# NTU-CompHydroMet-Lab/P2I-GAN-benchmark

Hardware: AMD Instinct MI355X
Metric: train frames/sec (128x128x16) (higher is better)
Workload: dtype f32

## Files before the change

### p2i-gan-benchmark_amd/csrc/conv.hip

```cpp
#include "conv_dma.h"

namespace p2i {


template <int MB, int NPIX, int WAVES_M, int CK>
__global__ __launch_bounds__(256) void patch_gemm_kernel(const PatchGeom g) {
  extern __shared__ __attribute__((aligned(16))) float smem[];
  constexpr int WAVES_N = 4 / WAVES_M;
  constexpr int TM = MB / (32 * WAVES_M);
  constexpr int TN = NPIX / (32 * WAVES_N);
  static_assert(TM >= 1 && TN >= 1, "tile too small");
  float* lw = smem;
  float* lp = smem + g.ntaps * CK * MB;

  const int tid = threadIdx.x, lane = tid & 63, wave = tid >> 6;
  const int wm = wave / WAVES_N, wn = wave % WAVES_N;
  const int l31 = lane & 31, lhi = lane >> 5;

  int tile = blockIdx.x;
  const int tw = tile % g.ntw; tile /= g.ntw;
  const int th = tile % g.nth; tile /= g.nth;
  const int tt = tile % g.ntt;
  const int tb = tile / g.ntt;
  const int j0b = tb << g.ljb, j0t = tt << g.ljt, j0h = th << g.ljh, j0w = tw << g.ljw;
// ... 104 lines not shown
          if (g.res) v += g.res[di];
          if (g.mask_y) v = act_grad(v, g.mask_y[di], g.mask_act);
          g.dst[di] = v;
        }
      }
    }
  }
}


typedef void (*patch_fn)(const PatchGeom);
template <int MB, int NPIX, int WM, int CK>
static int launch_patch(const PatchGeom& g, dim3 grid, size_t lds, hipStream_t s) {
  auto k = patch_gemm_kernel<MB, NPIX, WM, CK>;
  static bool attr_set = false;
  if (!attr_set) {
    (void)hipFuncSetAttribute((const void*)k, hipFuncAttributeMaxDynamicSharedMemorySize, 160 * 1024);
    attr_set = true;
  }
  P2I_LAUNCH(k, grid, dim3(256), lds, s, g);
  return launch_status();
}

static int dispatch_patch_dma(const TileCfg& c, int KG, const PatchGeom& g, dim3 grid, size_t lds, hipStream_t s) {
  int rc = dispatch_patch_dma_g0(c, KG, g, grid, lds, s);
  if (rc == -1) rc = dispatch_patch_dma_g1(c, KG, g, grid, lds, s);
  if (rc == -1) rc = dispatch_patch_dma_g2(c, KG, g, grid, lds, s);
  if (rc == -1) rc = dispatch_patch_dma_g3(c, KG, g, grid, lds, s);
  if (rc != -1) return rc;
  set_error("no DMA kernel instance for tile cfg %d %d %d %d kg %d", c.MB, c.NPIX, c.WM, c.CK, KG);
  return P2I_EINVAL;
}

static int dispatch_patch(const TileCfg& c, const PatchGeom& g, dim3 grid, size_t lds, hipStream_t s) {
#define P2I_CASE(mb_, npix_, wm_, ck_) \
  if (c.MB == mb_ && c.NPIX == npix_ && c.WM == wm_ && c.CK == ck_) return launch_patch<mb_, npix_, wm_, ck_>(g, grid, lds, s);
  P2I_CASE(128, 256, 2, 8)
  P2I_CASE(64, 256, 1, 8)
  P2I_CASE(64, 128, 2, 8)
  P2I_CASE(32, 128, 1, 8)
  P2I_CASE(128, 256, 2, 4)
  P2I_CASE(64, 256, 1, 4)
  P2I_CASE(64, 128, 2, 4)
  P2I_CASE(32, 128, 1, 4)
  P2I_CASE(128, 256, 2, 2)
  P2I_CASE(64, 256, 1, 2)
  P2I_CASE(64, 128, 2, 2)
  P2I_CASE(32, 128, 1, 2)
#undef P2I_CASE
  set_error("no kernel instance for tile cfg %d %d %d %d", c.MB, c.NPIX, c.WM, c.CK);
  return P2I_EINVAL;
}


static thread_local int g_last_plan[6] = {0, 0, 0, 0, 0, 0};

static int run_patch_gemm(PatchGeom g, const ClassSpec& cs, hipStream_t s);

static int run_patch_gemm_classes(PatchGeom g, const ClassSpec* css, int ncls, hipStream_t s) {
  if (g.src_y != nullptr || ncls > MAX_CLASSES) return 1;
  if (const X6Ctx& xc = x6_ctx(); xc.wb != nullptr) {
    bool all = true;
    for (int q = 0; q < ncls && all; ++q) all = run_patch_gemm_x6c(g, css[q], xc.wb, xc.ntaps_w, nullptr, s, true) == 0;
    if (all) {
      for (int q = 0; q < ncls; ++q)
        if (const int rc = run_patch_gemm_x6c(g, css[q], xc.wb, xc.ntaps_w, g_last_plan, s)) return rc == 1 ? P2I_EINVAL : rc;
      return P2I_OK;
    }
  }
  const ClassSpec& c0s = css[0];
  g.mT = c0s.mT; g.mH = c0s.mH; g.mW = c0s.mW;
  g.oT = c0s.oT; g.oH = c0s.oH; g.oW = c0s.oW;
  int lo[MAX_CLASSES][3], rng[3] = {0, 0, 0}, mx[3] = {0, 0, 0}, max_taps = 0;
  long long total_pix = 0;
  for (int q = 0; q < ncls; ++q) {
    const ClassSpec& cs = css[q];
    int hi[3] = {0, 0, 0};
    lo[q][0] = lo[q][1] = lo[q][2] = 0;
    for (int i = 0; i < cs.ntaps; ++i) {
      const int d[3] = {cs.dt[i], cs.dh[i], cs.dw[i]};
      for (int k = 0; k < 3; ++k) {
        if (i == 0 || d[k] < lo[q][k]) lo[q][k] = d[k];
        if (i == 0 || d[k] > hi[k]) hi[k] = d[k];
      }
    }
    for (int k = 0; k < 3; ++k) if (hi[k] - lo[q][k] > rng[k]) rng[k] = hi[k] - lo[q][k];
    if (cs.nT > mx[0]) mx[0] = cs.nT;
    if (cs.nH > mx[1]) mx[1] = cs.nH;
    if (cs.nW > mx[2]) mx[2] = cs.nW;
    if (cs.ntaps > max_taps) max_taps = cs.ntaps;
    total_pix += (long long)g.B * (cs.nT > 0 ? cs.nT : 0) * (cs.nH > 0 ? cs.nH : 0) * (cs.nW > 0 ? cs.nW : 0);
  }
  if (mx[0] <= 0 || mx[1] <= 0 || mx[2] <= 0) return P2I_OK;
  if (max_taps == 0) max_taps = 1;
  g.ntaps = max_taps;
  static const int cand[5][3] = {{128, 256, 2}, {64, 256, 1}, {128, 128, 2}, {64, 128, 2}, {32, 128, 1}};
  int best = -1, best_ck = 0;
  long long best_score = -1;
  PatchGeom bg = g;
  size_t best_lds = 0;
  dim3 best_grid;
  for (int ci = 0; ci < 5; ++ci) {
    const int MBc = cand[ci][0], NP = cand[ci][1];
    if (MBc > 32 && g.Cm <= MBc / 2) continue;
    int jb, jt, jh, jw;
    pick_tile_dims(NP, g.B, mx[0], mx[1], mx[2], jb, jt, jh, jw);
    PatchGeom t = g;
    t.ljb = ilog2(jb); t.ljt = ilog2(jt); t.ljh = ilog2(jh); t.ljw = ilog2(jw);
    t.eT = (jt - 1) * g.mT + rng[0] + 1;
    t.eH = (jh - 1) * g.mH + rng[1] + 1;
    t.eW = (jw - 1) * g.mW + rng[2] + 1;
    static const int v4_off = getenv("P2I_CONV_V4") ? (atoi(getenv("P2I_CONV_V4")) == 0) : 0;
    bool same_lo_w = true;
    for (int q = 1; q < ncls; ++q) same_lo_w = same_lo_w && lo[q][2] == lo[0][2];
    t.v4 = (!v4_off && same_lo_w && (g.sW & 3) == 0 && ((jw * g.mW) & 3) == 0) ? 1 : 0;
    t.v4sh = 0;
    if (t.v4) {
      t.v4sh = ((lo[0][2] % 4) + 4) % 4;
      t.eW = (t.eW + t.v4sh + 3) & ~3;
      t.eW4 = t.eW >> 2;
    }
    t.eWp = t.eW;
    t.eth = t.eT * t.eH;
    t.rpc = jb * t.eth;
    t.CSl = t.rpc * t.eW;
    t.CS = t.CSl;
    t.G4 = t.CSl >> 2;
    static const int force_ck16 = getenv("P2I_CONV_CK16") ? atoi(getenv("P2I_CONV_CK16")) : 0;
    for (int CKc = ((max_taps <= 4 || ((force_ck16 || g.Ck >= 256) && max_taps == 9 && MBc <= 64)) ? 16 : 8); CKc >= 2; CKc >>= 1) {
      if (g.Ck >= CKc ? (g.Ck % CKc != 0) : (CKc != 2 && g.Ck * 2 <= CKc)) continue;
      if (CKc == 2 && !(MBc == 64 && NP == 128) && !(MBc == 32)) continue;
      if ((CKc == 4 || CKc == 16) && MBc == 128 && NP == 128) continue;
      const int PT = CKc * t.CSl;
      if (PT >= 65536 || t.CSl >= 65536) continue;
      const int PTp = t.v4 ? (((PT >> 2) + 63) & ~63) * 4 : (PT + 63) & ~63;
      const int nwrows = max_taps * CKc;
      const size_t WSZ = (size_t)((nwrows * (MBc / 4) + 63) & ~63) * 4;
      const size_t lds = sizeof(float) * (((nwrows + 63) & ~63) + (size_t)PTp + 2 * (WSZ + PTp));
      if (lds > 160 * 1024) continue;
      const long long nb = (long long)ceil_div(g.Cm, MBc) * ((total_pix + NP - 1) / NP);
      long long score = (nb >= 256 ? 1000000000ll : nb * 1000000ll) + (long long)MBc * NP * 10 + CKc + (lds <= 80 * 1024 ? 5 : 0);
      if (score > best_score) {
        best_score = score; best = ci; best_ck = CKc; best_lds = lds;
        bg = t; bg.PT = PT;
        bg.ntt = ceil_div(mx[0], jt); bg.nth = ceil_div(mx[1], jh); bg.ntw = ceil_div(mx[2], jw);
        best_grid = dim3((unsigned)(ceil_div(g.B, jb) * bg.ntt * bg.nth * bg.ntw), (unsigned)ceil_div(g.Cm, MBc), (unsigned)ncls);
      }
      break;
    }
  }
  const unsigned long long sbytes = 4ull * g.B * g.Ck * g.sT * g.sH * g.sW;
  if (best < 0 || sbytes >= 0xF0000000ull) return 1;
  TileCfg c{cand[best][0], cand[best][1], cand[best][2], best_ck};
  bg.mg_csl = magic_u16(bg.CSl); bg.mg_ew = magic_u16(bg.eW);
  bg.mg_rpc = magic_u16(bg.rpc); bg.mg_eth = magic_u16(bg.eth); bg.mg_eh = magic_u16(bg.eH);
  if (bg.v4) { bg.mg_g4 = magic_u16(bg.G4); bg.mg_ew4 = magic_u16(bg.eW4); }
  bg.src_bytes = (unsigned)sbytes;
  bg.wp_bytes = g.wp_bytes;
  bg.nclass = ncls;
  for (int q = 0; q < ncls; ++q) {
    const ClassSpec& cs = css[q];
    ClassGeom& cgm = bg.cls[q];
    cgm.nT = cs.nT; cgm.nH = cs.nH; cgm.nW = cs.nW;
    cgm.pT = cs.pT; cgm.pH = cs.pH; cgm.pW = cs.pW;
    cgm.bT = lo[q][0]; cgm.bH = lo[q][1]; cgm.bW = lo[q][2];
    cgm.ntaps = cs.ntaps;
    for (int i = 0; i < cs.ntaps; ++i) {
      cgm.tap_w[i] = cs.tw[i];
      cgm.tap_off[i] = ((cs.dt[i] - lo[q][0]) * bg.eH + (cs.dh[i] - lo[q][1])) * bg.eW + (cs.dw[i] - lo[q][2]);
    }
  }
  bg.nT = css[0].nT; bg.nH = css[0].nH; bg.nW = css[0].nW;
  bg.pT = css[0].pT; bg.pH = css[0].pH; bg.pW = css[0].pW;
  bg.bT = lo[0][0]; bg.bH = lo[0][1]; bg.bW = lo[0][2];
  for (int i = 0; i < css[0].ntaps; ++i) { bg.tap_w[i] = bg.cls[0].tap_w[i]; bg.tap_off[i] = bg.cls[0].tap_off[i]; }
  if (bg.v4) {
    bg.bW -= bg.v4sh;
    for (int i = 0; i < css[0].ntaps; ++i) bg.tap_off[i] += bg.v4sh;
    for (int q = 0; q < ncls; ++q) {
      bg.cls[q].bW -= bg.v4sh;
      for (int i = 0; i < css[q].ntaps; ++i) bg.cls[q].tap_off[i] += bg.v4sh;
    }
  }
  if (ncls == 1) bg.ntaps = css[0].ntaps;
  const long long nb = (long long)best_grid.x * best_grid.y * best_grid.z;
  const int acc_regs = (c.MB / 32) * (c.NPIX / 32) / 4 * 16;
  const size_t red_bytes = (size_t)4 * acc_regs * 64 * 4;
  static const int kg27 = getenv("P2I_CONV_KG27") ? atoi(getenv("P2I_CONV_KG27")) : 1;
  const bool kg_27 = kg27 && max_taps == 27 && c.CK == 4 && ncls == 1;
  const int KG = ((nb <= 320 || (c.CK == 16 && max_taps == 9) || kg_27) && (c.CK >= 8 || kg_27) && c.MB <= 64 && red_bytes <= best_lds) ? 2 : 1;
  g_last_plan[0] = c.MB; g_last_plan[1] = c.NPIX; g_last_plan[2] = c.WM; g_last_plan[3] = c.CK;
  g_last_plan[4] = ncls > 1 ? 0 : ((max_taps == 9 && (c.CK <= 8 || KG == 2)) ? 9 : (max_taps == 1 ? 1 : ((max_taps == 27 && (c.CK == 4 || (c.CK < 4 && KG == 1))) ? 27 : 0)));
  g_last_plan[5] = KG;
  return dispatch_patch_dma(c, KG, bg, best_grid, best_lds, s);
}

static int run_patch_gemm(PatchGeom g, const ClassSpec& cs, hipStream_t s) {
  if (cs.nT <= 0 || cs.nH <= 0 || cs.nW <= 0) return P2I_OK;
  {
    const int rc = run_patch_gemm_classes(g, &cs, 1, s);
    if (rc != 1) return rc;
  }
  g.nT = cs.nT; g.nH = cs.nH; g.nW = cs.nW;
  g.mT = cs.mT; g.mH = cs.mH; g.mW = cs.mW;
  g.oT = cs.oT; g.oH = cs.oH; g.oW = cs.oW; g.pT = cs.pT; g.pH = cs.pH; g.pW = cs.pW;
  g.ntaps = cs.ntaps;
  g.nclass = 1;
  int lo[3] = {0, 0, 0}, hi[3] = {0, 0, 0};
  for (int i = 0; i < cs.ntaps; ++i) {
    const int d[3] = {cs.dt[i], cs.dh[i], cs.dw[i]};
    for (int k = 0; k < 3; ++k) {
      if (i == 0 || d[k] < lo[k]) lo[k] = d[k];
      if (i == 0 || d[k] > hi[k]) hi[k] = d[k];
    }
  }
  g.bT = lo[0]; g.bH = lo[1]; g.bW = lo[2];

  TileCfg c;
  c.CK = (g.Ck == 1) ? 2 : (cs.ntaps > 9 ? 4 : 8);
  if (g.Ck < c.CK && g.Ck > 1) c.CK = (g.Ck >= 4) ? 4 : 2;
  c.MB = g.Cm > 64 ? 128 : (g.Cm > 32 ? 64 : 32);
  c.NPIX = 256;
  const long long total_pix = (long long)g.B * cs.nT * cs.nH * cs.nW;
  auto nblocks = [&](const TileCfg& t) { return (long long)ceil_div(g.Cm, t.MB) * ((total_pix + t.NPIX - 1) / t.NPIX); };
  const long long want = 512;
  while (nblocks(c) < want) {
    if (c.MB == 128) { c.MB = 64; continue; }
    if (c.NPIX == 256) { c.NPIX = 128; continue; }
    if (c.MB == 64 && g.Cm > 32) { c.MB = 32; continue; }
    break;
  }
  if (c.MB == 128) { c.NPIX = 256; c.WM = 2; }
  else if (c.MB == 64) { c.WM = (c.NPIX == 256) ? 1 : 2; }
  else { c.NPIX = 128; c.WM = 1; }

  for (int attempt = 0; attempt < 4; ++attempt) {
    int jb, jt, jh, jw;
    pick_tile_dims(c.NPIX, g.B, cs.nT, cs.nH, cs.nW, jb, jt, jh, jw);
    g.ljb = ilog2(jb); g.ljt = ilog2(jt); g.ljh = ilog2(jh); g.ljw = ilog2(jw);
    g.eT = (jt - 1) * cs.mT + (hi[0] - lo[0]) + 1;
    g.eH = (jh - 1) * cs.mH + (hi[1] - lo[1]) + 1;
    g.eW = (jw - 1) * cs.mW + (hi[2] - lo[2]) + 1;
    g.eWp = g.eW | 1;
    g.eth = g.eT * g.eH;
    g.rpc = jb * g.eth;
    g.CS = g.rpc * g.eWp;
    g.mg_rpc = magic_u16(g.rpc); g.mg_eth = magic_u16(g.eth); g.mg_eh = magic_u16(g.eH);
    const size_t lds = sizeof(float) * ((size_t)cs.ntaps * c.CK * c.MB + (size_t)c.CK * g.CS);
    if (lds > 160 * 1024 || c.CK * g.rpc >= 65536) {
      if (c.CK > 2) { c.CK /= 2; continue; }
      if (c.NPIX == 256) { c.NPIX = 128; c.WM = (c.MB == 64) ? 2 : (c.MB == 128 ? 2 : 1); if (c.MB == 128) c.MB = 64; continue; }
      set_error("conv tile does not fit LDS (%zu bytes)", lds);
      return P2I_ELDS;
    }
    for (int i = 0; i < cs.ntaps; ++i) {
      g.tap_w[i] = cs.tw[i];
      g.tap_off[i] = ((cs.dt[i] - lo[0]) * g.eH + (cs.dh[i] - lo[1])) * g.eWp + (cs.dw[i] - lo[2]);
    }
    g.ntt = ceil_div(cs.nT, jt); g.nth = ceil_div(cs.nH, jh); g.ntw = ceil_div(cs.nW, jw);
    const int ntb = ceil_div(g.B, jb);
    dim3 grid((unsigned)(ntb * g.ntt * g.nth * g.ntw), (unsigned)ceil_div(g.Cm, c.MB));
    g_last_plan[0] = c.MB; g_last_plan[1] = c.NPIX; g_last_plan[2] = c.WM; g_last_plan[3] = c.CK; g_last_plan[4] = -1; g_last_plan[5] = 0;
    return dispatch_patch(c, g, grid, lds, s);
  }
  set_error("conv tile selection failed");
  return P2I_ELDS;
}

}

using namespace p2i;

#ifdef P2I_STAMP
namespace p2i { __device__ unsigned long long* p2i_stamp_buf = nullptr; }
extern "C" int p2i_debug_set_stamp(unsigned long long* buf) {
  return (int)hipMemcpyToSymbol(HIP_SYMBOL(p2i::p2i_stamp_buf), &buf, sizeof(buf));
}
#endif

extern "C" int p2i_conv_last_plan(int* out6) {
  if (!out6) return P2I_EINVAL;
  for (int i = 0; i < 6; ++i) out6[i] = g_last_plan[i];
  return P2I_OK;
}

extern "C" int p2i_conv_fwd(const p2i_conv_desc* d, const float* x, const float* wp, const float* bias,
                            const float* residual, float* y, int act, void* stream) {
  if (int e = check_desc(d)) return e;
  P2I_REQUIRE(x && wp && y, "null pointer");
  if (d->Cin == 1 && residual == nullptr && x6_ctx().wb == nullptr) {
    const int rc = c1_fwd(d, x, wp, bias, y, act, (hipStream_t)stream);
    if (rc != 1) { g_last_plan[0] = 32; g_last_plan[1] = 64; g_last_plan[2] = 1; g_last_plan[3] = 2; g_last_plan[4] = 27; g_last_plan[5] = 1; return rc; }
  }
  if (d->Cout == 1 && residual == nullptr) {
    const int rc = o1_fwd(d, x, wp, bias, y, act, (hipStream_t)stream);
    if (rc != 1) { g_last_plan[0] = 1; g_last_plan[1] = 64; g_last_plan[2] = 8; g_last_plan[3] = 1; g_last_plan[4] = 9; g_last_plan[5] = 3; return rc; }
  }
  PatchGeom g{};
  g.src = x; g.src_y = nullptr; g.wp = wp; g.bias = bias; g.res = residual; g.dst = y; g.act_epi = act; g.act_pro = P2I_ACT_NONE;
  g.B = d->B; g.Ck = d->Cin; g.Cm = d->Cout; g.CmPad = (d->Cout + 31) / 32 * 32;
  g.wp_bytes = 4u * (unsigned)(d->kt * d->kh * d->kw) * g.Ck * g.CmPad;
  g.sT = d->Ti; g.sH = d->Hi; g.sW = d->Wi; g.dT = d->To; g.dH = d->Ho; g.dW = d->Wo;
  ClassSpec cs{};
  cs.nT = d->To; cs.nH = d->Ho; cs.nW = d->Wo;
  cs.mT = d->st; cs.mH = d->sh; cs.mW = d->sw;
  cs.oT = cs.oH = cs.oW = 1; cs.pT = cs.pH = cs.pW = 0;
  int n = 0;
  for (int a = 0; a < d->kt; ++a)
    for (int b = 0; b < d->kh; ++b)
      for (int c = 0; c < d->kw; ++c) {
        cs.tw[n] = (short)n; cs.dt[n] = a - d->pt; cs.dh[n] = b - d->ph; cs.dw[n] = c - d->pw; ++n;
      }
  cs.ntaps = n;
  return run_patch_gemm(g, cs, (hipStream_t)stream);
}

extern "C" int p2i_conv_dgrad(const p2i_conv_desc* d, const float* dy, const float* y_act, int act,
                              const float* wp_d, const float* dx_add, const float* mask_y, int mask_act,
                              float* dx, void* stream) {
  if (int e = check_desc(d)) return e;
  P2I_REQUIRE(dy && wp_d && dx, "null pointer");
  PatchGeom g{};
  g.src = dy; g.src_y = y_act; g.wp = wp_d; g.bias = nullptr; g.res = dx_add; g.dst = dx; g.act_epi = P2I_ACT_NONE; g.act_pro = y_act ? act : P2I_ACT_NONE;
  g.mask_y = mask_y; g.mask_act = mask_y ? mask_act : P2I_ACT_NONE;
  P2I_REQUIRE(!(mask_y && y_act), "dgrad: use either the act'(y) prologue or the epilogue mask");
  if (d->Cin == 1 && !y_act && d->kt * d->kh * d->kw * d->Cout * 4 <= 64 * 1024)
    return c1_dgrad(d, dy, wp_d, dx_add, mask_y, mask_act, dx, (hipStream_t)stream);
  g.B = d->B; g.Ck = d->Cout; g.Cm = d->Cin; g.CmPad = (d->Cin + 31) / 32 * 32;
  g.wp_bytes = 4u * (unsigned)(d->kt * d->kh * d->kw) * g.Ck * g.CmPad;
  g.sT = d->To; g.sH = d->Ho; g.sW = d->Wo; g.dT = d->Ti; g.dH = d->Hi; g.dW = d->Wi;
  ClassSpec css[MAX_CLASSES];
  int ncls = 0;
  const bool mergeable = d->st * d->sh * d->sw <= MAX_CLASSES;
  for (int ct = 0; ct < d->st; ++ct)
    for (int chh = 0; chh < d->sh; ++chh)
      for (int cw = 0; cw < d->sw; ++cw) {
        ClassSpec cs{};
        cs.nT = (d->Ti - ct + d->st - 1) / d->st;
        cs.nH = (d->Hi - chh + d->sh - 1) / d->sh;
        cs.nW = (d->Wi - cw + d->sw - 1) / d->sw;
        cs.mT = cs.mH = cs.mW = 1;
        cs.oT = d->st; cs.oH = d->sh; cs.oW = d->sw; cs.pT = ct; cs.pH = chh; cs.pW = cw;
        int n = 0;
// ... 96 lines not shown
```

### p2i-gan-benchmark_amd/csrc/conv_common.h

```cpp
#pragma once
#include "common.h"

namespace p2i {

typedef float f32x16 __attribute__((ext_vector_type(16)));
constexpr int MAX_TAPS = 27;

typedef __attribute__((address_space(3))) void lds_void;
typedef int v4i32 __attribute__((ext_vector_type(4)));

__device__ __forceinline__ v4i32 make_rsrc(const void* p, unsigned bytes) {
  const unsigned long long a = (unsigned long long)p;
  v4i32 r;
  r[0] = __builtin_amdgcn_readfirstlane((int)(unsigned)a);
  r[1] = __builtin_amdgcn_readfirstlane((int)(unsigned)(a >> 32));
  r[2] = __builtin_amdgcn_readfirstlane((int)bytes);
  r[3] = 0x00020000;
  return r;
}
__device__ __forceinline__ unsigned lds_base(const float* shared_array) {
  return (unsigned)(size_t)(const lds_void*)shared_array;
}
__device__ __forceinline__ void dma_b32(const v4i32 rsrc, unsigned lds_addr, int voff, int soff) {
  const unsigned la = __builtin_amdgcn_readfirstlane(lds_addr);
// ... 7 lines not shown
  const int so = __builtin_amdgcn_readfirstlane(soff);
  unsigned keep;
  asm volatile("s_nop 4\n\ts_mov_b32 %0, m0\n\ts_mov_b32 m0, %2\n\ts_nop 0\n\tbuffer_load_dwordx4 %1, %3, %4 offen lds\n\ts_mov_b32 m0, %0"
               : "=&s"(keep) : "v"(voff), "s"(la), "s"(rsrc), "s"(so) : "memory");
}
__device__ __forceinline__ void dma_wait_all() { asm volatile("s_waitcnt vmcnt(0)" ::: "memory"); }


__device__ __forceinline__ void epilogue_tile16(const f32x16& acc, int o_base, int lhi, int Cm, bool pv, size_t pos_off, size_t chan_stride,
                                                const float* __restrict__ bias, int act_epi, const float* __restrict__ res,
                                                const float* __restrict__ mask_y, int mask_act, float* __restrict__ dst,
                                                bool atomic_out = false) {
#pragma unroll
  for (int h8 = 0; h8 < 2; ++h8) {
    int di[8];
    bool ok[8];
#pragma unroll
    for (int k = 0; k < 8; ++k) {
      const int r = h8 * 8 + k;
      const int o = o_base + (r & 3) + 8 * (r >> 2) + 4 * lhi;
      ok[k] = pv && o < Cm;
      di[k] = ok[k] ? (int)((size_t)o * chan_stride + pos_off) : 0;
    }
    float rv[8], mv[8];
    if (res) {
#pragma unroll
      for (int k = 0; k < 8; ++k) rv[k] = res[di[k]];
    }
    if (mask_y) {
#pragma unroll
      for (int k = 0; k < 8; ++k) mv[k] = mask_y[di[k]];
    }
#pragma unroll
    for (int k = 0; k < 8; ++k) {
      const int r = h8 * 8 + k;
      const int o = o_base + (r & 3) + 8 * (r >> 2) + 4 * lhi;
      float v = acc[r];
      if (bias) v += bias[o < Cm ? o : 0];
      v = act_apply(v, act_epi);
      if (res) v += rv[k];
      if (mask_y) v = act_grad(v, mv[k], mask_act);
      if (ok[k]) {
        if (atomic_out) atomicAdd(dst + di[k], v);
        else dst[di[k]] = v;
      }
    }
    __builtin_amdgcn_sched_barrier(0);
  }
}

typedef float f32x4e __attribute__((ext_vector_type(4)));
__device__ __forceinline__ void epilogue_tile16_v4(const f32x16& acc, float* __restrict__ tile_lds, int o_base, int lane, int Cm,
                                                   size_t pos4_off, bool pv4, size_t chan_stride,
                                                   const float* __restrict__ bias, int act_epi, const float* __restrict__ res,
                                                   const float* __restrict__ mask_y, int mask_act, float* __restrict__ dst, bool atomic_out = false) {
  constexpr int PITCH = 36;
  const int l31 = lane & 31, lhi = lane >> 5;
#pragma unroll
  for (int r = 0; r < 16; ++r) tile_lds[((r & 3) + 8 * (r >> 2) + 4 * lhi) * PITCH + l31] = acc[r];
  __builtin_amdgcn_fence(__ATOMIC_RELEASE, "wavefront");
  __builtin_amdgcn_wave_barrier();
  const int p4 = (lane & 7) * 4;
  int di[4];
  bool ok[4];
  f32x4e v[4], rv[4], mv[4];
#pragma unroll
  for (int k = 0; k < 4; ++k) {
    const int ch = k * 8 + (lane >> 3);
    const int o = o_base + ch;
    ok[k] = pv4 && o < Cm;
    di[k] = ok[k] ? (int)((size_t)o * chan_stride + pos4_off) : 0;
    v[k] = *reinterpret_cast<const f32x4e*>(tile_lds + ch * PITCH + p4);
  }
  if (res) {
#pragma unroll
    for (int k = 0; k < 4; ++k) rv[k] = *reinterpret_cast<const f32x4e*>(res + di[k]);
  }
  if (mask_y) {
#pragma unroll
    for (int k = 0; k < 4; ++k) mv[k] = *reinterpret_cast<const f32x4e*>(mask_y + di[k]);
  }
#pragma unroll
  for (int k = 0; k < 4; ++k) {
    const int o = o_base + k * 8 + (lane >> 3);
    const float bv = bias ? bias[o < Cm ? o : 0] : 0.f;
#pragma unroll
    for (int e = 0; e < 4; ++e) {
      float x = act_apply(v[k][e] + bv, act_epi);
      if (res) x += rv[k][e];
      if (mask_y) x = act_grad(x, mv[k][e], mask_act);
      v[k][e] = x;
    }
    if (ok[k]) {
      if (atomic_out) {
#pragma unroll
        for (int e = 0; e < 4; ++e) atomicAdd(dst + di[k] + e, v[k][e]);
      } else {
        *reinterpret_cast<f32x4e*>(dst + di[k]) = v[k];
      }
    }
  }
  __builtin_amdgcn_wave_barrier();
}

__device__ __forceinline__ void epilogue_pair16(const f32x16& acc0, const f32x16& acc1, int o_base, int lhi, int Cm, bool pv, size_t pos_off,
                                                size_t chan_stride, const float* __restrict__ res, const float* __restrict__ mask_y,
                                                int mask_act, float* __restrict__ dst, bool atomic_out = false) {
  typedef float f32x2e __attribute__((ext_vector_type(2)));
#pragma unroll
  for (int h4 = 0; h4 < 4; ++h4) {
    int di[4];
    bool ok[4];
#pragma unroll
    for (int k = 0; k < 4; ++k) {
      const int r = h4 * 4 + k;
      const int o = o_base + (r & 3) + 8 * (r >> 2) + 4 * lhi;
      ok[k] = pv && o < Cm;
      di[k] = ok[k] ? (int)((size_t)o * chan_stride + pos_off) : 0;
    }
    f32x2e rv[4], mv[4];
    if (res) {
#pragma unroll
      for (int k = 0; k < 4; ++k) rv[k] = *reinterpret_cast<const f32x2e*>(res + di[k]);
    }
    if (mask_y) {
#pragma unroll
      for (int k = 0; k < 4; ++k) mv[k] = *reinterpret_cast<const f32x2e*>(mask_y + di[k]);
    }
#pragma unroll
    for (int k = 0; k < 4; ++k) {
      const int r = h4 * 4 + k;
      f32x2e v;
      v[0] = acc0[r]; v[1] = acc1[r];
      if (res) { v[0] += rv[k][0]; v[1] += rv[k][1]; }
      if (mask_y) { v[0] = act_grad(v[0], mv[k][0], mask_act); v[1] = act_grad(v[1], mv[k][1], mask_act); }
      if (ok[k]) {
        if (atomic_out) { atomicAdd(dst + di[k], v[0]); atomicAdd(dst + di[k] + 1, v[1]); }
        else *reinterpret_cast<f32x2e*>(dst + di[k]) = v;
      }
    }
    __builtin_amdgcn_sched_barrier(0);
  }
}

static inline void pick_tile_dims(int NPIX, int B, int nT, int nH, int nW, int& jb, int& jt, int& jh, int& jw) {
  jw = pow2_ceil(nW); if (jw > 32) jw = 32;
  int rem = NPIX / jw;
  jh = pow2_ceil(nH); if (jh > rem) jh = rem;
  rem /= jh;
  jt = pow2_ceil(nT); if (jt > rem) jt = rem;
  rem /= jt;
  jb = rem;
  (void)B;
}


static inline int check_desc(const p2i_conv_desc* d) {
  P2I_REQUIRE(d != nullptr, "null conv desc");
  P2I_REQUIRE(d->B > 0 && d->Cin > 0 && d->Cout > 0, "bad channel/batch dims");
  P2I_REQUIRE(d->kt >= 1 && d->kh >= 1 && d->kw >= 1 && d->kt * d->kh * d->kw <= MAX_TAPS, "kernel taps > %d", MAX_TAPS);
  P2I_REQUIRE(d->st >= 1 && d->sh >= 1 && d->sw >= 1, "bad stride");
  P2I_REQUIRE(d->To == (d->Ti + 2 * d->pt - d->kt) / d->st + 1, "To inconsistent");
  P2I_REQUIRE(d->Ho == (d->Hi + 2 * d->ph - d->kh) / d->sh + 1, "Ho inconsistent");
  P2I_REQUIRE(d->Wo == (d->Wi + 2 * d->pw - d->kw) / d->sw + 1, "Wo inconsistent");
  const long long nin = (long long)d->B * d->Cin * d->Ti * d->Hi * d->Wi;
  const long long nout = (long long)d->B * d->Cout * d->To * d->Ho * d->Wo;
  P2I_REQUIRE(nin < (1ll << 31) && nout < (1ll << 31), "tensor too large for 32-bit indexing");
  return P2I_OK;
}


struct ClassGeom {
  int nT, nH, nW, pT, pH, pW, bT, bH, bW, ntaps;
  short tap_w[MAX_TAPS];
  int tap_off[MAX_TAPS];
};
constexpr int MAX_CLASSES = 8;

struct PatchGeom {
  const float* src;
  const float* src_y;
  const float* wp;
  const float* bias;
  const float* res;
  float* dst;
  int act_epi;
  int act_pro;
  int B, Ck, Cm, CmPad;
  int sT, sH, sW;
  int dT, dH, dW;
  int nT, nH, nW;
  int mT, mH, mW;
  int oT, oH, oW;
  int pT, pH, pW;
  int bT, bH, bW;
  int eT, eH, eW, eWp;
  int ljb, ljt, ljh, ljw;
  int ntt, nth, ntw;
  int ntaps;
  int CS;
  int rpc, eth;
  unsigned mg_rpc, mg_eth, mg_eh;
  short tap_w[MAX_TAPS];
  int tap_off[MAX_TAPS];
  const float* mask_y;
  int mask_act;
  int CSl;
  int PT;
  unsigned src_bytes, wp_bytes;
  unsigned mg_csl, mg_ew;
  int v4, v4sh;
  int eW4, G4;
  unsigned mg_g4, mg_ew4;
  const uint16_t* wb;
  unsigned wb_bytes;
  int ntaps_w;
  int TG, NTP, R;
  int ksplit;
  int pair_w;
  int nclass;
  ClassGeom cls[MAX_CLASSES];
};

struct ClassSpec {
  int nT, nH, nW;
  int mT, mH, mW;
  int oT, oH, oW, pT, pH, pW;
  int ntaps;
  short tw[MAX_TAPS];
  int dt[MAX_TAPS], dh[MAX_TAPS], dw[MAX_TAPS];
};

struct X6Ctx { const uint16_t* wb; int ntaps_w; };
X6Ctx& x6_ctx();

int run_patch_gemm_x6c(PatchGeom g, const ClassSpec& cs, const uint16_t* wb, int ntaps_w, int* plan6, hipStream_t s, bool dry = false);
int run_patch_gemm_x6c_fused(PatchGeom g, const ClassSpec* css, int ncls, const uint16_t* wb, int ntaps_w, int* plan6, hipStream_t s, bool dry = false);
bool x6c_would_take(const p2i_conv_desc* d, bool dgrad, int act_epi);

int run_patch_gemm_fused(PatchGeom g, const ClassSpec* css, int ncls, int* plan6, hipStream_t s);

int c1_dgrad(const p2i_conv_desc* d, const float* dy, const float* wp_d, const float* add, const float* mask_y, int mask_act,
             float* dx, hipStream_t s);
int c1_wgrad(const p2i_conv_desc* d, const float* x, const float* dy, float* dwp, float* dbias, hipStream_t s);
int c1_fwd(const p2i_conv_desc* d, const float* x, const float* wp, const float* bias, float* y, int act, hipStream_t s);
int o1_fwd(const p2i_conv_desc* d, const float* x, const float* wp, const float* bias, float* y, int act, hipStream_t s);

}
```

### p2i-gan-benchmark_amd/csrc/conv_dma.h

```cpp
#pragma once
#include "conv_common.h"

namespace p2i {

struct TileCfg { int MB, NPIX, WM, CK; };

#ifdef P2I_STAMP
extern __device__ unsigned long long* p2i_stamp_buf;
#endif

template <int MB, int NPIX, int WAVES_M, int CK, int NT, int KG>
__global__ __launch_bounds__(256 * KG) void patch_gemm_dma_kernel(const PatchGeom g) {
  extern __shared__ __attribute__((aligned(16))) float smem[];
  constexpr int WAVES_N = 4 / WAVES_M;
  constexpr int TM = MB / (32 * WAVES_M);
  constexpr int TN = NPIX / (32 * WAVES_N);
  constexpr int V = MB / 4;
  const bool multi = g.nclass > 1;
  const ClassGeom& cg = g.cls[multi ? blockIdx.z : 0];
  const int c_nT = multi ? cg.nT : g.nT, c_nH = multi ? cg.nH : g.nH, c_nW = multi ? cg.nW : g.nW;
  const int c_pT = multi ? cg.pT : g.pT, c_pH = multi ? cg.pH : g.pH, c_pW = multi ? cg.pW : g.pW;
  const int c_bT = multi ? cg.bT : g.bT, c_bH = multi ? cg.bH : g.bH, c_bW = multi ? cg.bW : g.bW;
  const int c_ntaps = multi ? cg.ntaps : g.ntaps;
  const short* c_tap_w = multi ? cg.tap_w : g.tap_w;
  const int* c_tap_off = multi ? cg.tap_off : g.tap_off;
  const int nwrows = g.ntaps * CK;
  const int WSZ = ((nwrows * V + 63) & ~63) * 4;
  const int PT4p = ((g.PT >> 2) + 63) & ~63;
  const int PTp = g.v4 ? PT4p * 4 : (g.PT + 63) & ~63;
  int* wtab = reinterpret_cast<int*>(smem);
  const int wtab_sz = (nwrows + 63) & ~63;
  int* ptab = wtab + wtab_sz;
  float* buf0 = smem + wtab_sz + PTp;
  const int BUFSZ = WSZ + PTp;

  constexpr int NTH = 256 * KG;
#ifdef P2I_STAMP
  unsigned long long st_entry;
  asm volatile("s_memtime %0\n\ts_waitcnt lgkmcnt(0)" : "=s"(st_entry) :: "memory");
#endif
  const int tid = threadIdx.x, lane = tid & 63, wave = (tid >> 6) & 3, kg = tid >> 8;
  const int wm = wave / WAVES_N, wn = wave % WAVES_N;
  const int l31 = lane & 31, lhi = lane >> 5;

  int tile = blockIdx.x;
  const int tw = tile % g.ntw; tile /= g.ntw;
  const int th = tile % g.nth; tile /= g.nth;
  const int tt = tile % g.ntt;
  const int tb = tile / g.ntt;
  const int j0b = tb << g.ljb, j0t = tt << g.ljt, j0h = th << g.ljh, j0w = tw << g.ljw;
  const int o0 = blockIdx.y * MB;
  const int JWm = (1 << g.ljw) - 1, JHm = (1 << g.ljh) - 1, JTm = (1 << g.ljt) - 1;
  const int sHW = g.sH * g.sW;
  const int src_t0 = j0t * g.mT + c_bT, src_h0 = j0h * g.mH + c_bH, src_w0 = j0w * g.mW + c_bW;

  for (int r = tid; r < wtab_sz; r += NTH) {
    int off = -4;
    if (r < nwrows) {
      const int tap = r / CK, c = r - tap * CK;
      if (tap < c_ntaps && c < g.Ck && o0 < g.CmPad) off = ((c_tap_w[tap] * g.Ck + c) * g.CmPad + o0) * 4;
    }
    wtab[r] = off;
  }
  if (g.v4) {
    for (int e = tid; e < PT4p; e += NTH) {
      int off = -16;
      if (e < (g.PT >> 2)) {
        const int c = fast_div(e, g.mg_g4);
        int rem = e - c * g.G4;
        const int row = g.eW4 == 1 ? rem : fast_div(rem, g.mg_ew4);
        const int g4 = rem - row * g.eW4;
        const int jb = fast_div(row, g.mg_eth);
        int r2 = row - jb * g.eth;
        const int et = fast_div(r2, g.mg_eh);
        const int eh = r2 - et * g.eH;
        const int b = j0b + jb, t = src_t0 + et, h = src_h0 + eh, w = src_w0 + 4 * g4;
        if (b < g.B && c < g.Ck && (unsigned)t < (unsigned)g.sT && (unsigned)h < (unsigned)g.sH && (unsigned)w < (unsigned)g.sW)
          off = ((((b * g.Ck + c) * g.sT + t) * sHW) + h * g.sW + w) * 4;
      }
      ptab[e] = off;
    }
  } else
  for (int e = tid; e < PTp; e += NTH) {
    int off = -4;
    if (e < g.PT) {
      const int c = fast_div(e, g.mg_csl);
      int rem = e - c * g.CSl;
      const int row = fast_div(rem, g.mg_ew);
      const int ew = rem - row * g.eW;
      const int jb = fast_div(row, g.mg_eth);
      int r2 = row - jb * g.eth;
      const int et = fast_div(r2, g.mg_eh);
      const int eh = r2 - et * g.eH;
      const int b = j0b + jb, t = src_t0 + et, h = src_h0 + eh, w = src_w0 + ew;
      if (b < g.B && c < g.Ck && (unsigned)t < (unsigned)g.sT && (unsigned)h < (unsigned)g.sH && (unsigned)w < (unsigned)g.sW)
        off = ((((b * g.Ck + c) * g.sT + t) * sHW) + h * g.sW + w) * 4;
    }
    ptab[e] = off;
  }

  int lane_base[TN];
#pragma unroll
  for (int f = 0; f < TN; ++f) {
    const int pix = (wn * TN + f) * 32 + l31;
    const int jw = pix & JWm;
    const int jh = (pix >> g.ljw) & JHm;
    const int jt = (pix >> (g.ljw + g.ljh)) & JTm;
    const int jb = pix >> (g.ljw + g.ljh + g.ljt);
    lane_base[f] = ((jb * g.eT + jt * g.mT) * g.eH + jh * g.mH) * g.eW + jw * g.mW + lhi * g.CSl;
  }
  f32x16 acc[TM][TN];
#pragma unroll
  for (int i = 0; i < TM; ++i)
#pragma unroll
    for (int f = 0; f < TN; ++f)
#pragma unroll
      for (int r = 0; r < 16; ++r) acc[i][f][r] = 0.f;

  const v4i32 rs_src = make_rsrc(g.src, g.src_bytes);
  const v4i32 rs_w = make_rsrc(g.wp, g.wp_bytes);
  const unsigned smem_la = lds_base(smem);
  const int buf0_off = (int)(buf0 - smem);
  const int chan_bytes = g.sT * sHW * 4;
  const int wbase = tid & ~63;
  const int nwv = nwrows * V;
  __syncthreads();

  constexpr int RW = 10, RP = 4;
  const int nwq = (((nwv + 63) & ~63) + NTH - 1) / NTH;
  const int npq = g.v4 ? (PT4p + NTH - 1) / NTH : RP + 1;
  const bool reg_issue = nwq <= RW && npq <= RP;
  int wv[RW], pv[RP];
  if (reg_issue) {
#pragma unroll
    for (int i = 0; i < RW; ++i) {
      const int f = i * NTH + tid;
      int voff = -4;
      if (i < nwq && f < nwv) {
        const int row = f / V, col4 = f - row * V;
        const int base = wtab[row];
        voff = base < 0 ? -4 : base + col4 * 16;
      }
      wv[i] = voff;
    }
#pragma unroll
    for (int i = 0; i < RP; ++i) {
      const int e = i * NTH + tid;
      pv[i] = (i < npq && e < PT4p) ? ptab[e] : -16;
    }
  }
  auto issue = [&](int c0, int bufoff) {
    const int w_soff = c0 * g.CmPad * 4;
    if (reg_issue) {
      const int p_soff = c0 * chan_bytes, pbo = bufoff + WSZ;
#pragma unroll
      for (int i = 0; i < RW; ++i)
        if (i < nwq && i * NTH + wbase < ((nwv + 63) & ~63))
          dma_b128(rs_w, smem_la + 4u * (bufoff + (i * NTH + wbase) * 4), wv[i], w_soff);
#pragma unroll
      for (int i = 0; i < RP; ++i)
        if (i < npq && i * NTH + wbase < PT4p)
          dma_b128(rs_src, smem_la + 4u * (pbo + (i * NTH + wbase) * 4), pv[i], p_soff);
      return;
    }
    for (int f0 = 0; f0 < nwv; f0 += NTH) {
      const int f = f0 + tid;
      int voff = -4;
      if (f < nwv) {
        const int row = f / V, col4 = f - row * V;
        const int base = wtab[row];
        voff = base < 0 ? -4 : base + col4 * 16;
      }
      if (f0 + wbase < ((nwv + 63) & ~63))
        dma_b128(rs_w, smem_la + 4u * (bufoff + (f0 + wbase) * 4), voff, w_soff);
    }
    const int pbo = bufoff + WSZ;
    const int p_soff = c0 * chan_bytes;
    if (g.v4) {
      for (int e0 = 0; e0 < PT4p; e0 += NTH) {
        const int e = e0 + tid;
        const int voff = e < PT4p ? ptab[e] : -16;
        if (e0 + wbase < PT4p)
          dma_b128(rs_src, smem_la + 4u * (pbo + (e0 + wbase) * 4), voff, p_soff);
      }
    } else
    for (int e0 = 0; e0 < PTp; e0 += NTH) {
      const int e = e0 + tid;
      const int voff = e < PTp ? ptab[e] : -4;
      if (e0 + wbase < PTp)
        dma_b32(rs_src, smem_la + 4u * (pbo + e0 + wbase), voff, p_soff);
    }
  };

  int toffs[NT > 0 ? NT : 1];
  if constexpr (NT > 0) {
#pragma unroll
    for (int t = 0; t < NT; ++t) toffs[t] = c_tap_off[t];
  }
  const int nchunks = (g.Ck + CK - 1) / CK;
#ifdef P2I_STAMP
  unsigned long long st_wait = 0, st_bar = 0, st_issue = 0, st_mfma = 0, st_t0, st_t1;
#define P2I_STAMP_NOW(v) do { __builtin_amdgcn_sched_barrier(0); asm volatile("s_memtime %0\n\ts_waitcnt lgkmcnt(0)" : "=s"(v) :: "memory"); __builtin_amdgcn_sched_barrier(0); } while (0)
  unsigned long long st_begin; P2I_STAMP_NOW(st_begin);
#endif
  issue(0, buf0_off);
  for (int k = 0; k < nchunks; ++k) {
#ifdef P2I_STAMP
    P2I_STAMP_NOW(st_t0);
#endif
    dma_wait_all();
#ifdef P2I_STAMP
    P2I_STAMP_NOW(st_t1); st_wait += st_t1 - st_t0;
#endif
    __syncthreads();
#ifdef P2I_STAMP
    P2I_STAMP_NOW(st_t0); st_bar += st_t0 - st_t1;
#endif
    float* cur = buf0 + (k & 1) * BUFSZ;
    if (k + 1 < nchunks) issue((k + 1) * CK, buf0_off + ((k + 1) & 1) * BUFSZ);
#ifdef P2I_STAMP
    P2I_STAMP_NOW(st_t1); st_issue += st_t1 - st_t0;
#endif
    const float* lw = cur + lhi * MB + wm * TM * 32 + l31;
    const float* lp = cur + WSZ;
    constexpr int NCP = CK / 2 / KG;
    float a[NCP][TM], bv[NCP][TN], an[NCP][TM], bn[NCP][TN];
    auto load_tap = [&](int tap, int toff, float (&aa)[NCP][TM], float (&bb)[NCP][TN]) {
#pragma unroll
      for (int cp = 0; cp < NCP; ++cp) {
#pragma unroll
        for (int i = 0; i < TM; ++i) aa[cp][i] = lw[tap * CK * MB + (kg * NCP + cp) * 2 * MB + i * 32];
#pragma unroll
        for (int f = 0; f < TN; ++f) bb[cp][f] = lp[lane_base[f] + toff + (kg * NCP + cp) * 2 * g.CSl];
      }
    };
    auto mfma_tap = [&](const float (&aa)[NCP][TM], const float (&bb)[NCP][TN]) {
#pragma unroll
      for (int cp = 0; cp < NCP; ++cp)
#pragma unroll
        for (int i = 0; i < TM; ++i)
#pragma unroll
          for (int f = 0; f < TN; ++f)
            acc[i][f] = __builtin_amdgcn_mfma_f32_32x32x2f32(aa[cp][i], bb[cp][f], acc[i][f], 0, 0, 0);
    };
    if constexpr (NT > 0) {
      load_tap(0, toffs[0], a, bv);
#pragma unroll
      for (int tap = 0; tap < NT; tap += 2) {
        if (tap + 1 < NT) load_tap(tap + 1, toffs[tap + 1 < NT ? tap + 1 : 0], an, bn);
        __builtin_amdgcn_sched_barrier(0);
        mfma_tap(a, bv);
        __builtin_amdgcn_sched_barrier(0);
        if (tap + 1 < NT) {
          if (tap + 2 < NT) load_tap(tap + 2, toffs[tap + 2 < NT ? tap + 2 : 0], a, bv);
          __builtin_amdgcn_sched_barrier(0);
          mfma_tap(an, bn);
          __builtin_amdgcn_sched_barrier(0);
        }
      }
    } else {
      const int nt = c_ntaps;
      if (nt > 0) load_tap(0, c_tap_off[0], a, bv);
// ... 107 lines not shown
```

Baseline: 11690.

## Add stride-2 conv replanning with lean tile dims and parity-split LDS patch layout

For single-class stride-2 (mW==2) convolutions, the host planner now re-picks tile dimensions to minimise the staged halo footprint. It can also store the LDS input patch with even and odd columns split and a padded row pitch chosen to reduce bank conflicts. The kernel's patch-table builder and lane base addressing are updated to use the padded pitch and the parity column mapping. The default mode (3) enables only the lean tile selection without parity, and keeps the vector path. This trades some extra host planning work and LDS footprint for less redundant staging and fewer LDS bank conflicts.

```diff
diff --git a/p2i-gan-benchmark_amd/csrc/conv.hip b/p2i-gan-benchmark_amd/csrc/conv.hip
--- a/p2i-gan-benchmark_amd/csrc/conv.hip
+++ b/p2i-gan-benchmark_amd/csrc/conv.hip
@@ -280,7 +280,8 @@
   const unsigned long long sbytes = 4ull * g.B * g.Ck * g.sT * g.sH * g.sW;
   if (best < 0 || sbytes >= 0xF0000000ull) return 1;
   TileCfg c{cand[best][0], cand[best][1], cand[best][2], best_ck};
-  bg.mg_csl = magic_u16(bg.CSl); bg.mg_ew = magic_u16(bg.eW);
+  bg.mg_csl = magic_u16(bg.CSl); bg.mg_ew = magic_u16(bg.eWp);
+  bg.par = 0; bg.eWh = 0;
   bg.mg_rpc = magic_u16(bg.rpc); bg.mg_eth = magic_u16(bg.eth); bg.mg_eh = magic_u16(bg.eH);
   if (bg.v4) { bg.mg_g4 = magic_u16(bg.G4); bg.mg_ew4 = magic_u16(bg.eW4); }
   bg.src_bytes = (unsigned)sbytes;
@@ -317,6 +318,54 @@
   static const int kg27 = getenv("P2I_CONV_KG27") ? atoi(getenv("P2I_CONV_KG27")) : 1;
   const bool kg_27 = kg27 && max_taps == 27 && c.CK == 4 && ncls == 1;
   const int KG = ((nb <= 320 || (c.CK == 16 && max_taps == 9) || kg_27) && (c.CK >= 8 || kg_27) && c.MB <= 64 && red_bytes <= best_lds) ? 2 : 1;
+  const char* s2e = getenv("P2I_CONV_S2");
+  const int s2 = s2e ? atoi(s2e) : 3;
+  if (s2 && ncls == 1 && c0s.mW == 2) {
+    PatchGeom t = bg;
+    int jb, jt, jh, jw;
+    if (s2 != 2) pick_tile_dims_lean(c.NPIX, g.B, mx[0], mx[1], mx[2], g.mT, g.mH, rng, jb, jt, jh, jw);
+    else pick_tile_dims(c.NPIX, g.B, mx[0], mx[1], mx[2], jb, jt, jh, jw);
+    t.ljb = ilog2(jb); t.ljt = ilog2(jt); t.ljh = ilog2(jh); t.ljw = ilog2(jw);
+    t.eT = (jt - 1) * g.mT + rng[0] + 1;
+    t.eH = (jh - 1) * g.mH + rng[1] + 1;
+    t.eW = (jw - 1) * g.mW + rng[2] + 1;
+    t.eWh = (t.eW + 1) / 2;
+    t.par = s2 != 3;
+    if (t.par) t.v4 = 0;
+    if (t.v4) { t.eW = (t.eW + t.v4sh + 3) & ~3; t.eW4 = t.eW >> 2; }
+    t.eWp = t.eW;
+    for (int p = t.eW, best_ways = 33; t.par && p < t.eW + 32; ++p) {
+      const int ways = patch_bank_ways(c.NPIX, t.ljw, t.ljh, t.ljt, t.eT, t.eH, p, g.mT, g.mH, 1);
+      if (ways < best_ways) { best_ways = ways; t.eWp = p; }
+    }
+    t.eth = t.eT * t.eH;
+    t.rpc = jb * t.eth;
+    t.CSl = t.rpc * t.eWp;
+    t.CS = t.CSl;
+    t.PT = c.CK * t.CSl;
+    const int nwrows = max_taps * c.CK;
+    t.G4 = t.CSl >> 2;
+    const size_t WSZ = (size_t)((nwrows * (c.MB / 4) + 63) & ~63) * 4;
+    const size_t PTp = t.v4 ? (size_t)(((t.PT >> 2) + 63) & ~63) * 4 : (size_t)((t.PT + 63) & ~63);
+    size_t lds = sizeof(float) * (((nwrows + 63) & ~63) + PTp + 2 * (WSZ + PTp));
+    if (KG == 2 && lds < red_bytes) lds = red_bytes;
+    if (t.PT < 65536 && lds <= 160 * 1024) {
+      t.ntt = ceil_div(mx[0], jt); t.nth = ceil_div(mx[1], jh); t.ntw = ceil_div(mx[2], jw);
+      t.bW = lo[0][2] - (t.v4 ? t.v4sh : 0); t.cls[0].bW = t.bW;
+      for (int i = 0; i < css[0].ntaps; ++i) {
+        const int dw = c0s.dw[i] - lo[0][2];
+        const int col = t.par ? ((dw & 1) ? t.eWh + dw / 2 : dw / 2) : dw + (t.v4 ? t.v4sh : 0);
+        t.tap_off[i] = ((c0s.dt[i] - lo[0][0]) * t.eH + (c0s.dh[i] - lo[0][1])) * t.eWp + col;
+        t.cls[0].tap_off[i] = t.tap_off[i];
+      }
+      t.mg_csl = magic_u16(t.CSl); t.mg_ew = magic_u16(t.eWp);
+      t.mg_rpc = magic_u16(t.rpc); t.mg_eth = magic_u16(t.eth); t.mg_eh = magic_u16(t.eH);
+      if (t.v4) { t.mg_g4 = magic_u16(t.G4); t.mg_ew4 = magic_u16(t.eW4); }
+      bg = t;
+      best_lds = lds;
+      best_grid = dim3((unsigned)(ceil_div(g.B, jb) * t.ntt * t.nth * t.ntw), best_grid.y, 1);
+    }
+  }
   g_last_plan[0] = c.MB; g_last_plan[1] = c.NPIX; g_last_plan[2] = c.WM; g_last_plan[3] = c.CK;
   g_last_plan[4] = ncls > 1 ? 0 : ((max_taps == 9 && (c.CK <= 8 || KG == 2)) ? 9 : (max_taps == 1 ? 1 : ((max_taps == 27 && (c.CK == 4 || (c.CK < 4 && KG == 1))) ? 27 : 0)));
   g_last_plan[5] = KG;
diff --git a/p2i-gan-benchmark_amd/csrc/conv_common.h b/p2i-gan-benchmark_amd/csrc/conv_common.h
--- a/p2i-gan-benchmark_amd/csrc/conv_common.h
+++ b/p2i-gan-benchmark_amd/csrc/conv_common.h
@@ -183,6 +183,36 @@
   rem /= jt;
   jb = rem;
   (void)B;
+}
+
+static inline void pick_tile_dims_lean(int NPIX, int B, int nT, int nH, int nW, int mT, int mH, const int rng[3], int& jb, int& jt,
+                                       int& jh, int& jw) {
+  jw = pow2_ceil(nW); if (jw > 32) jw = 32;
+  const int rem = NPIX / jw;
+  long long best = -1;
+  for (int h = pow2_ceil(nH) < rem ? pow2_ceil(nH) : rem; h >= 1; h >>= 1)
+    for (int t = pow2_ceil(nT) < rem / h ? pow2_ceil(nT) : rem / h; t >= 1; t >>= 1) {
+      const int b = rem / (h * t);
+      const long long tiles = (long long)ceil_div(B, b) * ceil_div(nT, t) * ceil_div(nH, h);
+      const long long staged = tiles * b * ((t - 1) * mT + rng[0] + 1) * ((h - 1) * mH + rng[1] + 1);
+      if (best < 0 || staged < best) { best = staged; jb = b; jt = t; jh = h; }
+    }
+}
+
+static inline int patch_bank_ways(int NPIX, int ljw, int ljh, int ljt, int eT, int eH, int eWp, int mT, int mH, int wstep) {
+  int worst = 1;
+  for (int p0 = 0; p0 < NPIX; p0 += 32) {
+    int cnt[32] = {0};
+    for (int l = 0; l < 32; ++l) {
+      const int pix = p0 + l;
+      const int w = pix & ((1 << ljw) - 1), h = (pix >> ljw) & ((1 << ljh) - 1), t = (pix >> (ljw + ljh)) & ((1 << ljt) - 1);
+      const int b = pix >> (ljw + ljh + ljt);
+      const int a = ((b * eT + t * mT) * eH + h * mH) * eWp + w * wstep;
+      const int k = ++cnt[a & 31];
+      if (k > worst) worst = k;
+    }
+  }
+  return worst;
 }
 
 
@@ -241,6 +271,7 @@
   unsigned src_bytes, wp_bytes;
   unsigned mg_csl, mg_ew;
   int v4, v4sh;
+  int par, eWh;
   int eW4, G4;
   unsigned mg_g4, mg_ew4;
   const uint16_t* wb;
diff --git a/p2i-gan-benchmark_amd/csrc/conv_dma.h b/p2i-gan-benchmark_amd/csrc/conv_dma.h
--- a/p2i-gan-benchmark_amd/csrc/conv_dma.h
+++ b/p2i-gan-benchmark_amd/csrc/conv_dma.h
@@ -87,13 +87,14 @@
       const int c = fast_div(e, g.mg_csl);
       int rem = e - c * g.CSl;
       const int row = fast_div(rem, g.mg_ew);
-      const int ew = rem - row * g.eW;
+      const int col = rem - row * g.eWp;
+      const int ew = g.par ? (col < g.eWh ? 2 * col : 2 * (col - g.eWh) + 1) : col;
       const int jb = fast_div(row, g.mg_eth);
       int r2 = row - jb * g.eth;
       const int et = fast_div(r2, g.mg_eh);
       const int eh = r2 - et * g.eH;
       const int b = j0b + jb, t = src_t0 + et, h = src_h0 + eh, w = src_w0 + ew;
-      if (b < g.B && c < g.Ck && (unsigned)t < (unsigned)g.sT && (unsigned)h < (unsigned)g.sH && (unsigned)w < (unsigned)g.sW)
+      if (ew < g.eW && b < g.B && c < g.Ck && (unsigned)t < (unsigned)g.sT && (unsigned)h < (unsigned)g.sH && (unsigned)w < (unsigned)g.sW)
         off = ((((b * g.Ck + c) * g.sT + t) * sHW) + h * g.sW + w) * 4;
     }
     ptab[e] = off;
@@ -107,7 +108,7 @@
     const int jh = (pix >> g.ljw) & JHm;
     const int jt = (pix >> (g.ljw + g.ljh)) & JTm;
     const int jb = pix >> (g.ljw + g.ljh + g.ljt);
-    lane_base[f] = ((jb * g.eT + jt * g.mT) * g.eH + jh * g.mH) * g.eW + jw * g.mW + lhi * g.CSl;
+    lane_base[f] = ((jb * g.eT + jt * g.mT) * g.eH + jh * g.mH) * g.eWp + (g.par ? jw : jw * g.mW) + lhi * g.CSl;
   }
   f32x16 acc[TM][TN];
 #pragma unroll
```

Result: no change. 11740 (median of 6 runs) (+0.4%).
